# josef-w/Differentiable-iLQR

Hardware: AMD Instinct MI355X
Metric: iLQR iters/sec (whole node), batch=65536 cartpole T=25 at 1/2/4/8 MI355X (higher is better)
Workload: dtype f32; 1 GPU; cartpole n=5 m=1 T=25, unconstrained iLQR, 65536 problems per GPU, step = one whole-batch MPC solve of lqr_iter=10 from u=0; batch_per_gpu=65536, global_batch=65536, T=25, lqr_iter=10, parallelism=batch-sharded x1 (no collective)

## Files before the change

differentiable-ilqr_amd/csrc/dilqr_fused.h:

```cpp
#pragma once
#include "dilqr_common.h"
#include "dilqr_launch.h"

namespace dilqr {

constexpr int TRAJ_AOS = 0, TRAJ_REC = 1;

template <int TL, int n, int m>
DEV void ld_xu(float (&x)[n], float (&u)[m], const float* __restrict__ xp, const float* __restrict__ up, size_t t,
               int B, int b) {
  const size_t tb = t * B + b;
  if constexpr (TL == TRAJ_REC) {
    float r[n + m];
    ld(r, (xp + (size_t)b * (n + m)) + t * (size_t)B * (n + m));
#pragma unroll
    for (int i = 0; i < n; ++i) x[i] = r[i];
#pragma unroll
    for (int a = 0; a < m; ++a) u[a] = r[n + a];
  } else {
    ld(x, xp + tb * n);
    ld(u, up + tb * m);
  }
}

template <int TL, int n, int m>
DEV void st_xu(float* __restrict__ xp, float* __restrict__ up, const float (&x)[n], const float (&u)[m], size_t t,
               int B, int b) {
  const size_t tb = t * B + b;
  if constexpr (TL == TRAJ_REC) {
    float r[n + m];
#pragma unroll
    for (int i = 0; i < n; ++i) r[i] = x[i];
#pragma unroll
    for (int a = 0; a < m; ++a) r[n + a] = u[a];
    st(xp + tb * (n + m), r);
  } else {
    st(xp + tb * n, x);
    st(up + tb * m, u);
  }
}

template <int d>
struct CostFull {
  static constexpr bool kDiag = false;
  static constexpr bool kSym = false;
  const float* __restrict__ C;
  const float* __restrict__ c;
  DEV void load(float (&Cr)[d][d], float (&cr)[d], size_t t, int B, int b) const {
    const size_t tb = t * B + b;
    ld2(Cr, C + tb * d * d); ld(cr, c + tb * d);
  }
};

template <int d>
constexpr int packed_cost_floats() { return d * (d + 1) / 2 + d; }
template <int d>
constexpr bool packed_diag_ok() { return (2 * d) % 4 == 0; }

constexpr unsigned char kCostSym = 1, kCostDiag = 2, kCostTinv = 4;

template <int d>
DEV void pack_cost(const float (&C)[d][d], const float (&c)[d], float (&buf)[packed_cost_floats<d>()], bool& sym,
                   bool& diag) {
  int k = 0;
#pragma unroll
  for (int i = 0; i < d; ++i) buf[k++] = C[i][i];
#pragma unroll
  for (int i = 0; i < d; ++i) buf[k++] = c[i];
  unsigned asym = 0u, offd = 0u;
#pragma unroll
  for (int i = 0; i < d; ++i)
#pragma unroll
    for (int j = i + 1; j < d; ++j) {
      asym |= __float_as_uint(C[i][j]) ^ __float_as_uint(C[j][i]);
      offd |= __float_as_uint(C[i][j]) | __float_as_uint(C[j][i]);
      buf[k++] = C[i][j];
    }
  sym &= asym == 0u;
  diag &= offd == 0u;
}

template <int K>
DEV bool same_bits(const float (&a)[K], const float (&b)[K]) {
  unsigned dif = 0u;
#pragma unroll
  for (int k = 0; k < K; ++k) dif |= __float_as_uint(a[k]) ^ __float_as_uint(b[k]);
  return dif == 0u;
}

template <int d, bool DIAG = false, bool TINV = false>
struct CostPacked {
  static constexpr bool kDiag = DIAG;
  static constexpr bool kSym = true;
  const float* __restrict__ P;
  int T;
  DEV void load(float (&Cr)[d][d], float (&cr)[d], size_t t_, int B, int b) const {
    constexpr int PK = packed_cost_floats<d>();
    const size_t t = TINV ? (size_t)(T - 1) : t_;
    if constexpr (DIAG) {
      static_assert(packed_diag_ok<d>(), "diagonal read needs whole float4 planes");
      constexpr int Q4 = SoaRec<PK>::Q4;
      const float4* q = reinterpret_cast<const float4*>(P);
      float buf[2 * d];
#pragma unroll
      for (int j = 0; j < 2 * d / 4; ++j) {
        float4 v = q[(t * Q4 + j) * B + b];
        buf[4 * j] = v.x; buf[4 * j + 1] = v.y; buf[4 * j + 2] = v.z; buf[4 * j + 3] = v.w;
      }
      const float z = 0.f;
#pragma unroll
      for (int i = 0; i < d; ++i) {
#pragma unroll
        for (int j = 0; j < d; ++j) Cr[i][j] = z;
        Cr[i][i] = buf[i];
        cr[i] = buf[d + i];
      }
    } else {
      float buf[PK];
      SoaRec<PK>::load(buf, P, T, t, B, b);
      int k = 2 * d;
#pragma unroll
      for (int i = 0; i < d; ++i) {
        Cr[i][i] = buf[i];
        cr[i] = buf[d + i];
      }
#pragma unroll
      for (int i = 0; i < d; ++i)
#pragma unroll
        for (int j = i + 1; j < d; ++j) { Cr[i][j] = buf[k]; Cr[j][i] = buf[k]; ++k; }
    }
  }
};

template <int d>
struct CostDiagConst {
  static constexpr bool kDiag = true;
  static constexpr bool kSym = true;
  float dg[d], cc[d];
  DEV void init(const float* __restrict__ P, int T, int B, int b) {
    float Cr[d][d], cr[d];
    CostPacked<d, true>{P, T}.load(Cr, cr, T - 1, B, b);
#pragma unroll
    for (int i = 0; i < d; ++i) { dg[i] = Cr[i][i]; cc[i] = cr[i]; }
  }
  template <int PK>
  DEV void set(const float (&pk)[PK]) {
#pragma unroll
    for (int i = 0; i < d; ++i) { dg[i] = pk[i]; cc[i] = pk[d + i]; }
  }
  DEV void load(float (&Cr)[d][d], float (&cr)[d], size_t, int, int) const {
    const float z = 0.f;
#pragma unroll
    for (int i = 0; i < d; ++i) {
#pragma unroll
      for (int j = 0; j < d; ++j) Cr[i][j] = z;
      Cr[i][i] = dg[i];
      cr[i] = cc[i];
    }
  }
};

template <class Model>
struct LaneCarry {
  static constexpr int n = Model::N, m = Model::M, d = n + m;
  float x0[n];
  CostDiagConst<d> cc;
  float u0[m], x1[n], u1[m];
  float xl[n], ul[m];
};

template <int m, int BM>
struct StepBounds {
  float lo[m], hi[m];
  DEV void load(const Bounds& bd, int t, int B, int b) {
    if constexpr (BM == DILQR_BOUNDS_TENSOR) {
      const size_t tb = (size_t)t * B + b;
      ld(lo, bd.lo_t + tb * m); ld(hi, bd.hi_t + tb * m);
    }
  }
  DEV float l(const Bounds& bd, int a) const {
    if constexpr (BM == DILQR_BOUNDS_TENSOR) return lo[a];
    else return bd.lo;
  }
  DEV float h(const Bounds& bd, int a) const {
    if constexpr (BM == DILQR_BOUNDS_TENSOR) return hi[a];
    else return bd.hi;
  }
};

template <int n, int m, int TL, int BM>
struct SweepIn {
  static constexpr int d = n + m;
  float C[d][d], c[d], x[n], u[m];
  StepBounds<m, BM> bnd;
  template <class CostT>
  DEV void load(const CostT& cs, const float* __restrict__ xp, const float* __restrict__ up, const Bounds& bd, int t,
                int B, int b) {
    cs.load(C, c, t, B, b); ld_xu<TL>(x, u, xp, up, t, B, b); bnd.load(bd, t, B, b);
  }
  template <class CostT>
  DEV void load_carried(const CostT& cs, const float (&xr)[n], const float (&ur)[m], const Bounds& bd, int t, int B,
                        int b) {
    cs.load(C, c, t, B, b); bnd.load(bd, t, B, b);
#pragma unroll
    for (int i = 0; i < n; ++i) x[i] = xr[i];
#pragma unroll
    for (int a = 0; a < m; ++a) u[a] = ur[a];
  }
};

struct GainRecs {
  float* p;
  int B, b;
};

template <int n, int m, int GREC, int TL, int BM>
struct FwdIn {
  static constexpr int d = n + m;
  float g[GREC], u[m], C[d][d], c[d], xnext[n], unext[m];
  StepBounds<m, BM> bnd;
  template <class CostT>
  DEV void load(const GainRecs& gr, const float* __restrict__ up, const CostT& cs,
                const float* __restrict__ xp, const Bounds& bd, int T, int t, int t1, int B, int b) {
    SoaRec<GREC>::load(g, gr.p, T, t, gr.B, gr.b); cs.load(C, c, t, B, b); bnd.load(bd, t, B, b);
    if constexpr (TL == TRAJ_REC) {
      ld_xu<TL>(xnext, unext, xp, up, t1, B, b);
    } else {
      ld(u, up + ((size_t)t * B + b) * m);
      ld(xnext, xp + ((size_t)t1 * B + b) * n);
    }
  }
  template <class CostT, class Carry>
  DEV void load_head(const GainRecs& gr, const CostT& cs, const Bounds& bd, const Carry& cy, int T, int B, int b) {
    SoaRec<GREC>::load(g, gr.p, T, 0, gr.B, gr.b); cs.load(C, c, 0, B, b); bnd.load(bd, 0, B, b);
#pragma unroll
    for (int i = 0; i < n; ++i) xnext[i] = cy.x1[i];
#pragma unroll
    for (int a = 0; a < m; ++a) { unext[a] = cy.u1[a]; u[a] = cy.u0[a]; }
  }
};

#ifndef DILQR_PF
#define DILQR_PF 2
#endif
constexpr int kPF = DILQR_PF;
#ifndef DILQR_PF_LS
#define DILQR_PF_LS 1
#endif
constexpr int kPFL = DILQR_PF_LS;
static_assert(kPFL == 1 || kPFL == 2, "the line search prefetches one or two steps ahead");

#ifndef DILQR_COPY_K
#define DILQR_COPY_K 5
#endif
constexpr int kCopyK = DILQR_COPY_K;

template <class Model, int BM, int TL, class CostT, bool PAIR = false, bool CARRY = false>
DEV int line_search(int T, int B, int b, const Model md, const float* __restrict__ x_init, const CostT& cs,
                    const float* __restrict__ x, const float* __restrict__ u, const Bounds& bd, float decay,
                    int max_ls, const GainRecs& ws, float* __restrict__ xa_out,
                    float* __restrict__ ua_out, float* __restrict__ xb_out, float* __restrict__ ub_out,
                    float* __restrict__ du_sq, float old_cost, float& cost_out, float& alpha_out,
                    bool b_in_gains = false, LaneCarry<Model>* cy = nullptr) {
  constexpr int n = Model::N, m = Model::M, d = n + m;
  constexpr int GREC = m * n + m;
  static_assert(!CARRY || TL == TRAJ_REC, "the carry hands over whole [x_t; u_t] records");
  f2 tl[d];
  static_assert(TL != TRAJ_REC || GREC == d, "B records in the gain slots need m = 1");
  if constexpr (PAIR) {
    max_ls = 2;
    b_in_gains = true;
  }
  float alpha = 1.f, cost = 0.f;
  int win = 0;
  for (int p = 0; p < max_ls; p += 2) {
    const bool twoB = p + 1 < max_ls;
    const float aA = alpha, aB = alpha * decay;
    const f2 al = {aA, aB};
    f2 xp[n], dp[n];
    {
      float x0[n];
      if constexpr (CARRY) {
#pragma unroll
        for (int i = 0; i < n; ++i) x0[i] = cy->x0[i];
      } else {
        ld(x0, x_init + (size_t)b * n);
      }
#pragma unroll
      for (int i = 0; i < n; ++i) { xp[i] = f2{x0[i], x0[i]}; dp[i] = f2{0.f, 0.f}; }
      if constexpr (TL == TRAJ_AOS) {
        st(xa_out + (size_t)b * n, x0);
        if (twoB) st(xb_out + (size_t)b * n, x0);
      }
    }
    f2 cp = {0.f, 0.f};
    auto cl = [T](int s) { return s < T ? s : T - 1; };
    FwdIn<n, m, GREC, TL, BM> cur, n1, n2;
    if constexpr (CARRY) {
      cur.load_head(ws, cs, bd, *cy, T, B, b);
    } else {
      cur.load(ws, u, cs, x, bd, T, 0, cl(1), B, b);
      if constexpr (TL == TRAJ_REC) {
        float x0r[n];
        ld_xu<TL>(x0r, cur.u, x, u, 0, B, b);
      }
    }
    if constexpr (kPFL >= 2) {
      if (T > 1) n1.load(ws, u, cs, x, bd, T, 1, cl(2), B, b);
    }
    auto step = [&](int t, auto last_c, auto& c, auto& nx) {
      constexpr bool LAST = decltype(last_c)::value;
      if constexpr (!LAST) {
        if constexpr (kPFL >= 2) {
          if (t + 2 < T) n2.load(ws, u, cs, x, bd, T, t + 2, cl(t + 3), B, b);
        } else {
          nx.load(ws, u, cs, x, bd, T, t + 1, cl(t + 2), B, b);
        }
      }
      f2 nu[m];
#pragma unroll
      for (int a = 0; a < m; ++a) {
        f2 sp = {0.f, 0.f};
#pragma unroll
        for (int j = 0; j < n; ++j) sp += c.g[a * n + j] * dp[j];
        nu[a] = (sp + c.u[a]) + al * c.g[m * n + a];
        if constexpr (BM != DILQR_BOUNDS_NONE) {
          const float lo = c.bnd.l(bd, a), hi = c.bnd.h(bd, a);
          nu[a] = f2{eclamp(nu[a].x, lo, hi), eclamp(nu[a].y, lo, hi)};
        }
      }
      {
        float ua[m], ub[m];
#pragma unroll
        for (int a = 0; a < m; ++a) { ua[a] = nu[a].x; ub[a] = nu[a].y; }
        if constexpr (TL == TRAJ_REC) {
          float xa[n], xb[n];
#pragma unroll
          for (int i = 0; i < n; ++i) { xa[i] = xp[i].x; xb[i] = xp[i].y; }
          st_xu<TL>(xa_out, nullptr, xa, ua, t, B, b);
          if (twoB) {
            if (b_in_gains) {
              float rb[d];
#pragma unroll
              for (int i = 0; i < n; ++i) rb[i] = xb[i];
#pragma unroll
              for (int a = 0; a < m; ++a) rb[n + a] = ub[a];
              SoaRec<d>::store(ws.p, rb, T, t, ws.B, ws.b);
            } else {
              st_xu<TL>(xb_out, nullptr, xb, ub, t, B, b);
            }
          }
        } else {
          st(ua_out + ((size_t)t * B + b) * m, ua);
          if (twoB) st(ub_out + ((size_t)t * B + b) * m, ub);
        }
      }
      if (p == 0) {
#pragma unroll
        for (int a = 0; a < m; ++a) {
          float e = c.u[a] - nu[a].x;
          du_sq[((size_t)t * m + a) * B + b] = e * e;
        }
      }
      f2 tau[d];
#pragma unroll
      for (int i = 0; i < n; ++i) tau[i] = xp[i];
#pragma unroll
      for (int a = 0; a < m; ++a) tau[n + a] = nu[a];
      cp += quad_cost<d, CostT::kDiag>(c.C, c.c, tau);
      if constexpr (CARRY && LAST) {
#pragma unroll
        for (int i = 0; i < d; ++i) tl[i] = tau[i];
      }
      if constexpr (!LAST) {
        f2 xnext[n];
        md.forward(xp, nu, xnext);
        float xa[n], xb[n];
#pragma unroll
        for (int i = 0; i < n; ++i) {
          dp[i] = xnext[i] - c.xnext[i];
          xp[i] = xnext[i];
          xa[i] = xnext[i].x;
          xb[i] = xnext[i].y;
        }
        if constexpr (TL == TRAJ_AOS) {
          st(xa_out + ((size_t)(t + 1) * B + b) * n, xa);
          if (twoB) st(xb_out + ((size_t)(t + 1) * B + b) * n, xb);
        }
      }
      if constexpr (!LAST) {
        if constexpr (TL == TRAJ_REC) {
#pragma unroll
          for (int a = 0; a < m; ++a) nx.u[a] = c.unext[a];
        }
      }
    };
    for (int t = 0; t < T - 1; ++t) {
      step(t, std::false_type{}, cur, n1);
      cur = n1;
      if constexpr (kPFL >= 2) n1 = n2;
#ifdef DILQR_STAMPS
      if (t == 0) DILQR_STAMP(9);
#endif
    }
    step(T - 1, std::true_type{}, cur, n1);
    DILQR_STAMP(10);
    const float cA = cp.x, cB = cp.y;
    if (!(cA > old_cost) || p == max_ls - 1) { cost = cA; alpha = aA; win = 0; break; }
    if (!(cB > old_cost) || p + 1 == max_ls - 1) { cost = cB; alpha = aB; win = 1; break; }
    alpha = aB * decay;
  }
  if constexpr (CARRY) {
#pragma unroll
    for (int i = 0; i < n; ++i) cy->xl[i] = win ? tl[i].y : tl[i].x;
#pragma unroll
    for (int a = 0; a < m; ++a) cy->ul[a] = win ? tl[n + a].y : tl[n + a].x;
  }
  if constexpr (TL == TRAJ_REC) {
    if (b_in_gains && win == 1) {
      auto copy_steps = [&](int t0, auto k_c) {
        constexpr int K = decltype(k_c)::value;
        float rb[K][d];
#pragma unroll
        for (int k = 0; k < K; ++k) SoaRec<d>::load(rb[k], ws.p, T, t0 + k, ws.B, ws.b);
#pragma unroll
        for (int k = 0; k < K; ++k) {
          float xt[n], ut[m];
#pragma unroll
          for (int i = 0; i < n; ++i) xt[i] = rb[k][i];
#pragma unroll
          for (int a = 0; a < m; ++a) ut[a] = rb[k][n + a];
          st_xu<TL>(xb_out, nullptr, xt, ut, t0 + k, B, b);
        }
      };
      int t = 0;
      for (; t + kCopyK <= T; t += kCopyK) copy_steps(t, std::integral_constant<int, kCopyK>{});
      for (; t < T; ++t) copy_steps(t, std::integral_constant<int, 1>{});
    }
  }
  DILQR_STAMP(11);
  cost_out = cost;
  alpha_out = alpha;
  return win;
}

template <class Model, int BM, int TL, bool ROLLOUT, class CostT, bool PREV = false, bool CARRY = false>
DEV int ilqr_problem(int T, int B, int b, const Model md, const float* __restrict__ x_init, const CostT& cs,
                     float* __restrict__ pack_out, unsigned char* __restrict__ sym_out, const float* __restrict__ x,
                     const float* __restrict__ u, const Bounds& bd, float decay, int max_ls,
                     const GainRecs& ws, float* __restrict__ xa_out, float* __restrict__ ua_out,
                     float* __restrict__ xb_out, float* __restrict__ ub_out, float* __restrict__ du_sq,
                     float& cost_out, float& alpha_out, bool b_in_gains = false,
                     float prev_cost = 0.f, unsigned* flags_out = nullptr, LaneCarry<Model>* cy = nullptr) {
  constexpr int n = Model::N, m = Model::M, d = n + m;
  constexpr int MODE = BM == DILQR_BOUNDS_NONE ? GAIN_UNC : GAIN_BOX;
  constexpr int GREC = m * n + m;
  constexpr int PK = packed_cost_floats<d>();
  float old_cost = 0.f;
  if constexpr (PREV) old_cost = prev_cost;
  bool sym = true, diag = true, tinv = true;
  bool symsofar = true;
  float pk_last[PK];
  {
    RiccatiState<n, m> rs;
    rs.init();
    float xn[n];
#pragma unroll
    for (int i = 0; i < n; ++i) xn[i] = 0.f;
    SweepIn<n, m, TL, BM> cur, n1, n2;
    if constexpr (CARRY) cur.load_carried(cs, cy->xl, cy->ul, bd, T - 1, B, b);
    else cur.load(cs, x, u, bd, T - 1, B, b);
    if constexpr (kPF >= 2) n1.load(cs, x, u, bd, T > 1 ? T - 2 : 0, B, b);
    const int t_head = T > 1 ? 1 : 0;
    using SI = SweepIn<n, m, TL, BM>;
    auto sweep_body = [&](int t, auto last_c, const SI& cur, float (&g)[GREC]) {
      constexpr bool LAST = decltype(last_c)::value;
      float tau[d], Ctau[d], cb[d];
#pragma unroll
      for (int i = 0; i < n; ++i) tau[i] = cur.x[i];
#pragma unroll
      for (int a = 0; a < m; ++a) tau[n + a] = cur.u[a];
      if (pack_out) {
        float buf[PK];
        pack_cost(cur.C, cur.c, buf, sym, diag);
        if constexpr (LAST) {
          SoaRec<PK>::store(pack_out, buf, T, t, B, b);
#pragma unroll
          for (int k = 0; k < PK; ++k) pk_last[k] = buf[k];
        } else {
          const bool same = same_bits(buf, pk_last);
          if (tinv && !same)
            for (int s = t + 1; s < T - 1; ++s) SoaRec<PK>::store(pack_out, pk_last, T, s, B, b);
          tinv &= same;
          if (!tinv) SoaRec<PK>::store(pack_out, buf, T, t, B, b);
        }
      }
      float obj = 0.f;
      if constexpr (PREV) c_tau<d, CostT::kDiag>(cur.C, tau, Ctau);
      else obj = quad_cost<d, CostT::kDiag>(cur.C, cur.c, tau, Ctau);
#pragma unroll
      for (int i = 0; i < d; ++i) cb[i] = Ctau[i] + cur.c[i];
      float Ft[n][d];
      if constexpr (!LAST) {
        if constexpr (ROLLOUT && Model::kJacFromNext) md.jacobian_next(cur.x, cur.u, xn, Ft);
        else md.jacobian(cur.x, cur.u, Ft);
      } else {
#pragma unroll
        for (int i = 0; i < n; ++i)
#pragma unroll
          for (int j = 0; j < d; ++j) Ft[i][j] = 0.f;
      }
      float zIt[m], lb[m], ub[m];
#pragma unroll
      for (int a = 0; a < m; ++a) {
        zIt[a] = 0.f; lb[a] = 0.f; ub[a] = 0.f;
        if constexpr (MODE == GAIN_BOX) {
          lb[a] = cur.bnd.l(bd, a) - cur.u[a];
          ub[a] = cur.bnd.h(bd, a) - cur.u[a];
        }
      }
      float Kt[m][n], kt[m];
      using FS = typename Model::FSparsity;
      if constexpr (CostT::kSym) {
        rs.template step<MODE, FS, CostT::kDiag, true>(cur.C, cb, Ft, zIt, lb, ub, Kt, kt);
      } else {
        symsofar &= bitwise_symmetric(cur.C);
        if (symsofar) rs.template step<MODE, FS, CostT::kDiag, true>(cur.C, cb, Ft, zIt, lb, ub, Kt, kt);
        else rs.template step<MODE, FS, CostT::kDiag, false>(cur.C, cb, Ft, zIt, lb, ub, Kt, kt);
      }
#pragma unroll
      for (int a = 0; a < m; ++a) {
#pragma unroll
        for (int j = 0; j < n; ++j) g[a * n + j] = Kt[a][j];
        g[m * n + a] = kt[a];
      }
      if constexpr (!PREV) old_cost += obj;
#pragma unroll
      for (int i = 0; i < n; ++i) xn[i] = cur.x[i];
      if constexpr (CARRY) {
        if (t == t_head) {
#pragma unroll
          for (int i = 0; i < n; ++i) cy->x1[i] = cur.x[i];
#pragma unroll
          for (int a = 0; a < m; ++a) cy->u1[a] = cur.u[a];
        }
#pragma unroll
        for (int a = 0; a < m; ++a) cy->u0[a] = cur.u[a];
      }
    };
    auto sweep_step = [&](int t, auto last_c) {
      if constexpr (kPF >= 2) n2.load(cs, x, u, bd, t > 1 ? t - 2 : 0, B, b);
      else n1.load(cs, x, u, bd, t > 0 ? t - 1 : 0, B, b);
      float g[GREC];
      sweep_body(t, last_c, cur, g);
      SoaRec<GREC>::store(ws.p, g, T, t, ws.B, ws.b);
      cur = n1;
      if constexpr (kPF >= 2) n1 = n2;
    };
    sweep_step(T - 1, std::true_type{});
    DILQR_STAMP(8);
#ifndef DILQR_SWEEP_UNROLL
#define DILQR_SWEEP_UNROLL 2
#endif
#pragma unroll DILQR_SWEEP_UNROLL
    for (int t = T - 2; t >= 0; --t) sweep_step(t, std::false_type{});
    if constexpr (CARRY) {
#pragma unroll
      for (int i = 0; i < n; ++i) cy->x0[i] = xn[i];
    }
    if (sym_out) {
      const unsigned char f = sym ? (unsigned char)(kCostSym | (diag && packed_diag_ok<d>() ? kCostDiag : 0) |
                                                    (tinv ? kCostTinv : 0))
                                  : 0;
      sym_out[b] = f;
      if (flags_out) *flags_out = f;
    }
  }
  DILQR_STAMP(2);
  if constexpr (!CostT::kDiag && packed_diag_ok<d>()) {
    if (pack_out && sym && diag && tinv) {
      CostDiagConst<d> cc;
      cc.set(pk_last);
      if (b_in_gains && max_ls == 2)
        return line_search<Model, BM, TL, CostDiagConst<d>, true, CARRY>(T, B, b, md, x_init, cc, x, u, bd, decay,
                                                                         max_ls, ws, xa_out, ua_out, xb_out, ub_out,
                                                                         du_sq, old_cost, cost_out, alpha_out,
                                                                         b_in_gains, cy);
      return line_search<Model, BM, TL, CostDiagConst<d>, false, CARRY>(T, B, b, md, x_init, cc, x, u, bd, decay,
                                                                        max_ls, ws, xa_out, ua_out, xb_out, ub_out,
                                                                        du_sq, old_cost, cost_out, alpha_out,
                                                                        b_in_gains, cy);
    }
  }
  if (b_in_gains && max_ls == 2)
    return line_search<Model, BM, TL, CostT, true, CARRY>(T, B, b, md, x_init, cs, x, u, bd, decay, max_ls, ws, xa_out,
                                                          ua_out, xb_out, ub_out, du_sq, old_cost, cost_out,
                                                          alpha_out, b_in_gains, cy);
  return line_search<Model, BM, TL, CostT, false, CARRY>(T, B, b, md, x_init, cs, x, u, bd, decay, max_ls, ws, xa_out,
                                                         ua_out, xb_out, ub_out, du_sq, old_cost, cost_out, alpha_out,
                                                         b_in_gains, cy);
}

template <class Model, int BM>
__global__ void __launch_bounds__(kBlock) k_ilqr_iterate(int T, int B, const float* __restrict__ theta,
                                                         const float* __restrict__ x_init, const float* __restrict__ C,
                                                         const float* __restrict__ c, const float* __restrict__ x,
                                                         const float* __restrict__ u, Bounds bd, float decay, int max_ls,
                                                         float* __restrict__ ws, float* __restrict__ x_out,
                                                         float* __restrict__ u_out, float* __restrict__ cost_out,
                                                         float* __restrict__ du_sq, float* __restrict__ alpha_out,
                                                         const dilqr_mpc_ctrl* __restrict__ ctrl) {
  if (ctrl && ctrl->stopped) return;
  int b = blockIdx.x * blockDim.x + threadIdx.x;
  if (b >= B) return;
  constexpr int n = Model::N, m = Model::M;
  constexpr int GREC = m * n + m;
  Model md; md.load(theta);
  float cost, alpha;
  float* xb = ws + (size_t)T * B * GREC;
  float* ub = xb + (size_t)T * B * n;
  const int win = ilqr_problem<Model, BM, TRAJ_AOS, false>(T, B, b, md, x_init, CostFull<n + m>{C, c}, nullptr, nullptr, x, u,
                                                   bd, decay,
                                            max_ls, GainRecs{ws, B, b},
                                            x_out, u_out, xb, ub, du_sq, cost, alpha);
  if (win) {
    for (int t = 0; t < T; ++t) {
      const size_t tb = (size_t)t * B + b;
      float xt[n], ut[m];
      ld(xt, xb + tb * n); ld(ut, ub + tb * m);
      st(x_out + tb * n, xt); st(u_out + tb * m, ut);
    }
  }
  cost_out[b] = cost;
  alpha_out[b] = alpha;
}

using MpcState = dilqr_mpc_state;
constexpr int kSlots = 4;

DEV bool mpc_decide(const MpcState& S, int B, int k, int G, float eps, int not_improved_lim);

DEV void free_slots(int cur, int best, int& sa, int& sb) {
  sa = -1;
  sb = -1;
#pragma unroll
  for (int s = 0; s < kSlots; ++s) {
    const bool fr = s != cur && s != best;
    sb = (fr && sa >= 0 && sb < 0) ? s : sb;
    sa = (fr && sa < 0) ? s : sa;
  }
}

struct LaneIter {
  float cost, alpha;
  int slot;
};

template <class Model, int BM, bool LG, bool FIRST, bool PREV = true, int GS = kBlock, bool CARRY = false,
          bool ONLY_DC = false>
DEV LaneIter mpc_iteration_lane(int T, int B, int b, const Model md, const float* __restrict__ x_init,
                                const float* __restrict__ C, const float* __restrict__ c, const Bounds& bd,
                                float decay, int max_ls, const MpcState& S, float* __restrict__ du_sq,
                                float* __restrict__ lds_gains, int cur, int best, unsigned pk, float prev_cost,
                                unsigned* flags_out = nullptr, LaneCarry<Model>* cy = nullptr) {
  constexpr int n = Model::N, m = Model::M;
  const size_t TBd = (size_t)T * B * (n + m);
  int sa, sb;
  free_slots(cur, best, sa, sb);
  const float* xcur = S.Xs + cur * TBd;
  float* xsa = S.Xs + sa * TBd;
  float* xsb = S.Xs + sb * TBd;
  float cost, alpha;
  int win;
  const GainRecs gr = LG ? GainRecs{lds_gains, GS, (int)threadIdx.x} : GainRecs{S.ws, B, b};
  const CostFull<n + m> full{C, c};
  const bool b_lds = LG && max_ls <= 2;
  if constexpr (FIRST) {
    win = ilqr_problem<Model, BM, TRAJ_REC, true>(T, B, b, md, x_init, full, S.Cpk, S.Cpk ? S.cost_sym : nullptr,
                                                  xcur, nullptr, bd, decay, max_ls, gr, xsa, nullptr, xsb, nullptr,
                                                  du_sq, cost, alpha, b_lds, 0.f, flags_out);
  } else {
    if (ONLY_DC || (pk & (kCostDiag | kCostTinv)) == (kCostDiag | kCostTinv)) {
      if constexpr (packed_diag_ok<n + m>()) {
        CostDiagConst<n + m> cc;
        if constexpr (CARRY) cc = cy->cc;
        else cc.init(S.Cpk, T, B, b);
        win = ilqr_problem<Model, BM, TRAJ_REC, true, CostDiagConst<n + m>, PREV, CARRY>(T, B, b, md, x_init, cc, nullptr, nullptr, xcur, nullptr, bd,
                                                      decay, max_ls, gr, xsa, nullptr, xsb, nullptr, du_sq, cost,
                                                      alpha, b_lds, prev_cost, nullptr, cy);
      } else {
        __builtin_unreachable();
      }
    } else if constexpr (ONLY_DC) {
      __builtin_unreachable();
    } else if (pk & kCostDiag) {
      if constexpr (packed_diag_ok<n + m>())
        win = ilqr_problem<Model, BM, TRAJ_REC, true, CostPacked<n + m, true>, PREV, CARRY>(T, B, b, md, x_init, CostPacked<n + m, true>{S.Cpk, T}, nullptr,
                                                      nullptr, xcur, nullptr, bd, decay, max_ls, gr, xsa, nullptr, xsb,
                                                      nullptr, du_sq, cost, alpha, b_lds, prev_cost, nullptr, cy);
      else
        __builtin_unreachable();
    } else if ((pk & (kCostSym | kCostTinv)) == (kCostSym | kCostTinv))
      win = ilqr_problem<Model, BM, TRAJ_REC, true, CostPacked<n + m, false, true>, PREV, CARRY>(T, B, b, md, x_init, CostPacked<n + m, false, true>{S.Cpk, T},
                                                    nullptr, nullptr, xcur, nullptr, bd, decay, max_ls, gr, xsa, nullptr,
                                                    xsb, nullptr, du_sq, cost, alpha, b_lds, prev_cost, nullptr, cy);
    else if (pk & kCostSym)
      win = ilqr_problem<Model, BM, TRAJ_REC, true, CostPacked<n + m>, PREV, CARRY>(T, B, b, md, x_init, CostPacked<n + m>{S.Cpk, T}, nullptr, nullptr,
                                                    xcur, nullptr, bd, decay, max_ls, gr, xsa, nullptr, xsb, nullptr,
                                                    du_sq, cost, alpha, b_lds, prev_cost, nullptr, cy);
    else
      win = ilqr_problem<Model, BM, TRAJ_REC, true, CostFull<n + m>, PREV, CARRY>(T, B, b, md, x_init, full, nullptr, nullptr, xcur, nullptr, bd,
                                                    decay, max_ls, gr, xsa, nullptr, xsb, nullptr, du_sq, cost,
                                                    alpha, b_lds, prev_cost, nullptr, cy);
  }
  return LaneIter{cost, alpha, win ? sb : sa};
}

DEV bool mpc_takes_best(bool first, float cost, float best_cost, float best_cost_eps) {
  return first || cost <= best_cost + best_cost_eps;
}

template <class Model, int BM, bool LG, bool FIRST>
__global__ void __launch_bounds__(kBlock) k_mpc_iterate(int T, int B, const float* __restrict__ theta,
                                                        const float* __restrict__ x_init, const float* __restrict__ C,
                                                        const float* __restrict__ c, Bounds bd, float decay, int max_ls,
                                                        int iteration, float best_cost_eps, float eps,
                                                        int not_improved_lim, int G, MpcState S) {
  constexpr bool first = FIRST;
  int b = blockIdx.x * blockDim.x + threadIdx.x;
  const int bl = b < B ? b : B - 1;
  const int cur = S.slot[bl], best = S.slot[B + bl];
  const unsigned char pk = (!FIRST && S.Cpk) ? S.cost_sym[bl] : 0;
  const float prev = FIRST ? 0.f : S.cost[bl];
  const float best_cost = FIRST ? 0.f : S.best_cost[bl];
  DILQR_STAMP(0);
  DILQR_STAMP(6);
  if (mpc_decide(S, B, iteration, G, eps, not_improved_lim)) return;
  if (b >= B) return;
  DILQR_STAMP(1);
  Model md; md.load(theta);
  extern __shared__ __attribute__((aligned(16))) float lds_gains[];
  const LaneIter r = mpc_iteration_lane<Model, BM, LG, FIRST>(T, B, b, md, x_init, C, c, bd, decay, max_ls, S,
                                                              S.du_sq, lds_gains, cur, best, pk, prev);
  DILQR_STAMP(3);
  S.cost[b] = r.cost;
  S.alpha[b] = r.alpha;
  const bool take = mpc_takes_best(first, r.cost, best_cost, best_cost_eps);
  if (take) {
    S.best_cost[b] = r.cost;
    S.slot[B + b] = (unsigned char)r.slot;
  }
  S.improved[b] = take ? (first ? 1 : 2) : 0;
  if (S.best_iter && take) S.best_iter[b] = iteration;
  S.slot[b] = (unsigned char)r.slot;
  DILQR_STAMP(4);
  DILQR_STAMP(7);
}

DEV int sync_gmax(int B) { return (B + 63) / 64; }

DEV bool mpc_decide(const MpcState& S, int B, int k, int G, float eps, int not_improved_lim) {
  if (k == 0) return false;
  if (G < 0) return false;
  const int gm = sync_gmax(B), par = (k - 1) & 1;
  const unsigned* pm = S.done_counter + 16 + (2 * par) * gm;
  const unsigned* pa = S.done_counter + 16 + (2 * par + 1) * gm;
  const int lane = threadIdx.x & 63;
  const dilqr_mpc_ctrl in = S.ctrl[(k - 1) & 1];
  unsigned mx = 0u;
  int any = 0;
  if ((gm & 3) == 0 && G <= 1024) {
    const uint4* pm4 = reinterpret_cast<const uint4*>(pm);
    const uint4* pa4 = reinterpret_cast<const uint4*>(pa);
    uint4 vm[4], va[4];
#pragma unroll
    for (int j = 0; j < 4; ++j) {
      const int i = lane + 64 * j;
      const bool ok = 4 * i < G;
      vm[j] = ok ? pm4[i] : make_uint4(0u, 0u, 0u, 0u);
      va[j] = ok ? pa4[i] : make_uint4(0u, 0u, 0u, 0u);
    }
#pragma unroll
    for (int j = 0; j < 4; ++j) {
      const int i0 = 4 * (lane + 64 * j);
      const unsigned e[4] = {vm[j].x, vm[j].y, vm[j].z, vm[j].w};
      const unsigned f[4] = {va[j].x, va[j].y, va[j].z, va[j].w};
#pragma unroll
      for (int q = 0; q < 4; ++q) {
        if (i0 + q < G) {
          mx = e[q] > mx ? e[q] : mx;
          any |= (int)f[q];
        }
      }
    }
  } else {
    for (int i = lane; i < G; i += 64) {
      unsigned v = pm[i];
      mx = v > mx ? v : mx;
      any |= (int)pa[i];
    }
  }
  dilqr_mpc_ctrl out = in;
  if (!in.stopped) {
    const bool all_below = __ballot(!(__uint_as_float(mx) < eps)) == 0ull;
    const bool any_imp = __ballot(any != 0) != 0ull;
    out.iter = in.iter + 1;
    out.n_not_improved = any_imp ? 0 : in.n_not_improved + 1;
    if (all_below || out.n_not_improved > not_improved_lim) out.stopped = 1;
    if (blockIdx.x == 0) {
#pragma unroll
      for (int off = 32; off > 0; off >>= 1) {
        unsigned o = __shfl_xor(mx, off, 64);
        mx = o > mx ? o : mx;
      }
      out.max_du_bits = mx;
    }
  }
  if (blockIdx.x == 0 && threadIdx.x == 0) S.ctrl[k & 1] = out;
  return out.stopped != 0;
}

template <class Model>
constexpr int slot_layout() { return Model::N + Model::M <= 8 ? TRAJ_REC : TRAJ_AOS; }
constexpr int slot_layout_nm(int n, int m) { return n + m <= 8 ? TRAJ_REC : TRAJ_AOS; }

#ifndef DILQR_BEGIN_PF
#define DILQR_BEGIN_PF 1
#endif
template <class Model, bool ANALYSE = false, bool CARRY = false>
DEV unsigned mpc_begin_lane(int T, int B, int b, const Model& md, const float* __restrict__ x_init,
                            const float* __restrict__ u_init, const MpcState& S,
                            const float* __restrict__ C = nullptr, const float* __restrict__ c = nullptr,
                            LaneCarry<Model>* cy = nullptr) {
  constexpr int n = Model::N, m = Model::M, d = n + m;
  constexpr int PK = packed_cost_floats<d>();
  S.slot[b] = 0; S.slot[B + b] = 0;
  constexpr int TL = slot_layout<Model>();
  const CostFull<d> full{C, c};
  constexpr int PFB = ANALYSE ? DILQR_BEGIN_PF : 1;
  float Cq[PFB][d][d], cq[PFB][d], uq[PFB][m];
  auto load_step = [&](int s, int t) {
    if (u_init) {
      ld(uq[s], u_init + ((size_t)t * B + b) * m);
    } else {
#pragma unroll
      for (int a = 0; a < m; ++a) uq[s][a] = 0.f;
    }
    if constexpr (ANALYSE) full.load(Cq[s], cq[s], t, B, b);
  };
#pragma unroll
  for (int s = 0; s < PFB; ++s) load_step(s, s < T ? s : T - 1);
  bool sym = true, diag = true, tinv = true;
  float pk_first[PK];
  float xt[n];
  ld(xt, x_init + (size_t)b * n);
  for (int t0 = 0; t0 < T; t0 += PFB) {
#pragma unroll
    for (int s = 0; s < PFB; ++s) {
      const int t = t0 + s;
      if (t >= T) break;
      float ut[m], xn[n];
      float Cc[d][d], cc[d];
#pragma unroll
      for (int a = 0; a < m; ++a) ut[a] = uq[s][a];
      if constexpr (ANALYSE) {
#pragma unroll
        for (int i = 0; i < d; ++i) {
          cc[i] = cq[s][i];
#pragma unroll
          for (int j = 0; j < d; ++j) Cc[i][j] = Cq[s][i][j];
        }
      }
      const int tp = t + PFB < T ? t + PFB : T - 1;
      load_step(s, tp);
      st_xu<TL>(S.Xs, S.Us, xt, ut, t, B, b);
      if constexpr (CARRY) {
#pragma unroll
        for (int a = 0; a < m; ++a) cy->ul[a] = ut[a];
      }
      if (t < T - 1) {
        md.forward(xt, ut, xn);
#pragma unroll
        for (int i = 0; i < n; ++i) xt[i] = xn[i];
      }
      if constexpr (ANALYSE) {
        float buf[PK];
        pack_cost(Cc, cc, buf, sym, diag);
        if (t == 0) {
#pragma unroll
          for (int k = 0; k < PK; ++k) pk_first[k] = buf[k];
        } else {
          const bool same = same_bits(buf, pk_first);
          if (tinv && !same)
            for (int s_ = 0; s_ < t; ++s_) SoaRec<PK>::store(S.Cpk, pk_first, T, s_, B, b);
          tinv &= same;
          if (!tinv) SoaRec<PK>::store(S.Cpk, buf, T, t, B, b);
        }
      }
    }
  }
  if constexpr (CARRY) {
#pragma unroll
    for (int i = 0; i < n; ++i) cy->xl[i] = xt[i];
    if constexpr (ANALYSE && packed_diag_ok<d>()) cy->cc.set(pk_first);
  }
  if constexpr (ANALYSE) {
    if (tinv) SoaRec<PK>::store(S.Cpk, pk_first, T, T - 1, B, b);
    const unsigned char f = sym ? (unsigned char)(kCostSym | (diag && packed_diag_ok<d>() ? kCostDiag : 0) |
                                                  (tinv ? kCostTinv : 0))
                                : 0;
    S.cost_sym[b] = f;
    return f;
  }
  return 0u;
}

constexpr int kDenseCount = 9;

DEV void mpc_reset_ctrl(const MpcState& S) {
  dilqr_mpc_ctrl z = {};
  S.ctrl[0] = z;
  S.ctrl[1] = z;
#pragma unroll
  for (int i = 0; i <= kDenseCount; ++i) S.done_counter[i] = 0u;
}

#ifndef DILQR_SOLVE_LPW
#define DILQR_SOLVE_LPW 64
#endif
#ifndef DILQR_SOLVE_OCC
#define DILQR_SOLVE_OCC 1
#endif
constexpr int kSolveLpw = DILQR_SOLVE_LPW;

template <class Model, int BM, bool LG>
__global__ void __launch_bounds__(kBlock, DILQR_SOLVE_OCC) k_mpc_solve_fixed(int T, int B, const float* __restrict__ theta,
                                                            const float* __restrict__ x_init,
                                                            const float* __restrict__ u_init,
                                                            const float* __restrict__ C, const float* __restrict__ c,
                                                            Bounds bd, float decay, int max_ls, int iters,
                                                            float best_cost_eps, MpcState S) {
  constexpr int m = Model::M;
  const int b = blockIdx.x * kSolveLpw + threadIdx.x;
  DILQR_STAMP(0);
  DILQR_STAMP(6);
  if (b == 0) mpc_reset_ctrl(S);
  if (b >= B || (int)threadIdx.x >= kSolveLpw) return;
  Model md; md.load(theta);
  extern __shared__ __attribute__((aligned(16))) float lds_gains[];
  LaneCarry<Model> cy;
  const unsigned pk = S.Cpk ? mpc_begin_lane<Model, true, true>(T, B, b, md, x_init, u_init, S, C, c, &cy)
                            : mpc_begin_lane<Model, false, true>(T, B, b, md, x_init, u_init, S, nullptr, nullptr, &cy);
  DILQR_STAMP(1);
  LaneIter r{0.f, 0.f, 0};
  int cur = 0, best = 0, best_iter = 0;
  float best_cost = 0.f;
  bool take = true;
  const size_t plane = (size_t)T * m * B;
  auto iterate = [&](auto only_dc) {
    constexpr bool DC = decltype(only_dc)::value;
    r = mpc_iteration_lane<Model, BM, LG, false, false, kSolveLpw, true, DC>(T, B, b, md, x_init, C, c, bd, decay,
                                                                             max_ls, S, S.du_sq, lds_gains, 0, 0, pk,
                                                                             0.f, nullptr, &cy);
    cur = best = r.slot;
    best_cost = r.cost;
    DILQR_STAMP(3);
    for (int it = 1; it < iters; ++it) {
      if (it == iters - 1) DILQR_STAMP(4);
      r = mpc_iteration_lane<Model, BM, LG, false, true, kSolveLpw, true, DC>(T, B, b, md, x_init, C, c, bd, decay,
                                                                              max_ls, S, S.du_sq + it * plane,
                                                                              lds_gains, cur, best, pk, r.cost,
                                                                              nullptr, &cy);
      take = mpc_takes_best(false, r.cost, best_cost, best_cost_eps);
      if (take) { best_cost = r.cost; best = r.slot; best_iter = it; }
      cur = r.slot;
    }
  };
  bool wave_dc = false;
  if constexpr (packed_diag_ok<Model::N + m>())
    wave_dc = __ballot((pk & (kCostDiag | kCostTinv)) != (kCostDiag | kCostTinv)) == 0ull;
  if (wave_dc) iterate(std::true_type{});
  else iterate(std::false_type{});
  S.cost[b] = r.cost;
  S.alpha[b] = r.alpha;
  S.best_cost[b] = best_cost;
  S.slot[b] = (unsigned char)cur;
  S.slot[B + b] = (unsigned char)best;
  S.improved[b] = take ? (iters == 1 ? 1 : 2) : 0;
  S.best_iter[b] = best_iter;
  DILQR_STAMP(5);
  DILQR_STAMP(7);
}

constexpr int kSmallMax = 256;

template <class Model, int BM, bool LG>
__global__ void __launch_bounds__(kSmallMax) k_mpc_solve_small(int T, int B, const float* __restrict__ theta,
                                                               const float* __restrict__ x_init,
                                                               const float* __restrict__ u_init,
                                                               const float* __restrict__ C,
                                                               const float* __restrict__ c, Bounds bd, float decay,
                                                               int max_ls, int iters, float best_cost_eps, float eps,
                                                               int not_improved_lim, MpcState S) {
  constexpr int m = Model::M;
  __shared__ unsigned red_max[kSmallMax / 64];
  __shared__ int red_any[kSmallMax / 64];
  extern __shared__ __attribute__((aligned(16))) float lds_gains[];
  const int b = threadIdx.x;
  const bool act = b < B;
  const int nw = (int)(blockDim.x + 63) / 64, w = b >> 6;
  const int TM = T * m;
  Model md; md.load(theta);
  unsigned pk = 0u;
  LaneIter r{0.f, 0.f, 0};
  int cur = 0, best = 0, imp = 0;
  float best_cost = 0.f;
  if (act) {
    pk = S.Cpk ? mpc_begin_lane<Model, true>(T, B, b, md, x_init, u_init, S, C, c)
               : mpc_begin_lane<Model>(T, B, b, md, x_init, u_init, S);
    r = mpc_iteration_lane<Model, BM, LG, false, false, 64>(T, B, b, md, x_init, C, c, bd, decay, max_ls, S,
                                                            S.du_sq, lds_gains, 0, 0, pk, 0.f);
    cur = best = r.slot;
    best_cost = r.cost;
    imp = 1;
  }
  int done = 0, n_not_improved = 0, stopped = 0;
  unsigned mx_all = 0u, mx_prev = 0u;
  for (;;) {
    ++done;
    __syncthreads();
    unsigned mx = 0u;
    int any = 0;
    if (act) {
      float s2 = 0.f;
      const float* p = S.du_sq + (size_t)b * TM;
      for (int i = 0; i < TM; ++i) s2 += p[i];
      const float fdn = sqrtf(s2);
      S.full_du_norm[b] = fdn;
      if (imp) S.best_du[b] = fdn;
      mx = __float_as_uint(fdn);
      any = imp == 2;
    }
#pragma unroll
    for (int off = 32; off > 0; off >>= 1) {
      const unsigned o = __shfl_xor(mx, off, 64);
      mx = o > mx ? o : mx;
      any |= __shfl_xor(any, off, 64);
    }
    if ((b & 63) == 0) { red_max[w] = mx; red_any[w] = any; }
    __syncthreads();
    mx = 0u;
    any = 0;
    for (int i = 0; i < nw; ++i) { mx = red_max[i] > mx ? red_max[i] : mx; any |= red_any[i]; }
    mx_prev = mx_all;
    mx_all = mx;
    if (done == iters) break;
    n_not_improved = any ? 0 : n_not_improved + 1;
    if (__uint_as_float(mx) < eps || n_not_improved > not_improved_lim) {
      stopped = 1;
      break;
    }
    if (act) {
      r = mpc_iteration_lane<Model, BM, LG, false, true, 64>(T, B, b, md, x_init, C, c, bd, decay, max_ls, S,
                                                             S.du_sq, lds_gains, cur, best, pk, r.cost);
      const bool take = mpc_takes_best(false, r.cost, best_cost, best_cost_eps);
      if (take) { best_cost = r.cost; best = r.slot; }
      imp = take ? 2 : 0;
      cur = r.slot;
    }
  }
  if (act) {
    S.cost[b] = r.cost;
    S.alpha[b] = r.alpha;
    S.best_cost[b] = best_cost;
    S.slot[b] = (unsigned char)cur;
    S.slot[B + b] = (unsigned char)best;
    S.improved[b] = imp;
  }
  if (b == 0) {
    dilqr_mpc_ctrl o = {};
    o.iter = stopped ? done : done - 1;
    o.stopped = stopped;
    o.n_not_improved = n_not_improved;
    o.max_du_bits = stopped ? mx_all : mx_prev;
    S.ctrl[0] = o;
    S.ctrl[1] = o;
  }
}

inline bool lds_gains_fit(size_t lds, int B) {
  if (lds > 65536) return false;
  if (lds * 4 <= kLdsPerCU) return true;
  static int cus = [] {
    int dev = 0, n = 0;
    if (hipGetDevice(&dev) != hipSuccess ||
        hipDeviceGetAttribute(&n, hipDeviceAttributeMultiprocessorCount, dev) != hipSuccess)
      return 0;
    return n;
  }();
  return (size_t)grid_for(B) <= (size_t)cus * (kLdsPerCU / lds);
}
template <class MD>
int launch_mpc_step_tpp(const MpcStepArgs& a) {
#define LAUNCH_IT(BM_, LG_, FIRST_, LDS_)                                                                     \
  k_mpc_iterate<MD, BM_, LG_, FIRST_><<<grid_for(a.B), kBlock, LDS_, a.stream>>>(                            \
      a.T, a.B, a.theta, a.x_init, a.C, a.c, a.bd, a.decay, a.max_ls, a.iteration, a.best_cost_eps, a.eps, a.lim, \
      a.G, a.st)
#define LAUNCH_MPC(BM_)                                                                                      \
  do {                                                                                                       \
    const size_t lds = (size_t)a.T * kBlock * (MD::N * MD::M + MD::M) * sizeof(float);                      \
    const bool lg = lds_gains_fit(lds, a.B);                                                                 \
    if (a.iteration == 0 && lg) LAUNCH_IT(BM_, true, true, lds);                                             \
    else if (a.iteration == 0) LAUNCH_IT(BM_, false, true, 0);                                               \
    else if (lg) LAUNCH_IT(BM_, true, false, lds);                                                           \
    else LAUNCH_IT(BM_, false, false, 0);                                                                    \
  } while (0)
  if (a.bd.mode == DILQR_BOUNDS_TENSOR) LAUNCH_MPC(DILQR_BOUNDS_TENSOR);
  else if (a.bd.mode != DILQR_BOUNDS_NONE) LAUNCH_MPC(DILQR_BOUNDS_SCALAR);
  else LAUNCH_MPC(DILQR_BOUNDS_NONE);
#undef LAUNCH_MPC
#undef LAUNCH_IT
  return launched();
}

template <class MD>
int launch_mpc_solve_tpp(const MpcSolveArgs& a) {
#define LAUNCH_SOLVE(BM_)                                                                                    \
  do {                                                                                                       \
    const size_t lds = (size_t)a.T * kSolveLpw * (MD::N * MD::M + MD::M) * sizeof(float);                   \
    const int grid = (int)(((long long)a.B + kSolveLpw - 1) / kSolveLpw);                                   \
    if (lds_gains_fit(lds * kBlock / kSolveLpw, a.B))                                                       \
      k_mpc_solve_fixed<MD, BM_, true><<<grid, kBlock, lds, a.stream>>>(                                      \
          a.T, a.B, a.theta, a.x_init, a.u_init, a.C, a.c, a.bd, a.decay, a.max_ls, a.iters, a.best_cost_eps, a.st); \
    else                                                                                                     \
      k_mpc_solve_fixed<MD, BM_, false><<<grid, kBlock, 0, a.stream>>>(                                       \
          a.T, a.B, a.theta, a.x_init, a.u_init, a.C, a.c, a.bd, a.decay, a.max_ls, a.iters, a.best_cost_eps, a.st); \
  } while (0)
  if (a.bd.mode == DILQR_BOUNDS_TENSOR) LAUNCH_SOLVE(DILQR_BOUNDS_TENSOR);
  else if (a.bd.mode != DILQR_BOUNDS_NONE) LAUNCH_SOLVE(DILQR_BOUNDS_SCALAR);
  else LAUNCH_SOLVE(DILQR_BOUNDS_NONE);
#undef LAUNCH_SOLVE
  return launched();
}

template <class MD>
int launch_mpc_solve_small_tpp(const MpcSolveArgs& a, float eps, int lim) {
  if (a.B > kSmallMax) return DILQR_E_SHAPE;
  const int threads = (a.B + 63) / 64 * 64;
  const size_t lds = (size_t)a.T * 64 * (MD::N * MD::M + MD::M) * sizeof(float);
  const bool lg = threads == 64 && lds <= 65536;
#define LAUNCH_SMALL(BM_)                                                                                    \
  do {                                                                                                       \
    if (lg)                                                                                                  \
      k_mpc_solve_small<MD, BM_, true><<<1, threads, lds, a.stream>>>(                                        \
          a.T, a.B, a.theta, a.x_init, a.u_init, a.C, a.c, a.bd, a.decay, a.max_ls, a.iters, a.best_cost_eps, eps, \
          lim, a.st);                                                                                        \
    else                                                                                                     \
      k_mpc_solve_small<MD, BM_, false><<<1, threads, 0, a.stream>>>(                                         \
          a.T, a.B, a.theta, a.x_init, a.u_init, a.C, a.c, a.bd, a.decay, a.max_ls, a.iters, a.best_cost_eps, eps, \
          lim, a.st);                                                                                        \
  } while (0)
  if (a.bd.mode == DILQR_BOUNDS_TENSOR) LAUNCH_SMALL(DILQR_BOUNDS_TENSOR);
  else if (a.bd.mode != DILQR_BOUNDS_NONE) LAUNCH_SMALL(DILQR_BOUNDS_SCALAR);
  else LAUNCH_SMALL(DILQR_BOUNDS_NONE);
#undef LAUNCH_SMALL
  return launched();
}

template <class MD>
int launch_ilqr_iterate_tpp(const IlqrIterArgs& a) {
#define LAUNCH_IT(BM_)                                                                                        \
  k_ilqr_iterate<MD, BM_><<<grid_for(a.B), kBlock, 0, a.stream>>>(a.T, a.B, a.theta, a.x_init, a.C, a.c, a.x, a.u, \
                                                                   a.bd, a.decay, a.max_ls, a.ws, a.x_out,     \
                                                                   a.u_out, a.cost, a.du_sq, a.alpha, a.ctrl)
  if (a.bd.mode == DILQR_BOUNDS_TENSOR) LAUNCH_IT(DILQR_BOUNDS_TENSOR);
  else if (a.bd.mode != DILQR_BOUNDS_NONE) LAUNCH_IT(DILQR_BOUNDS_SCALAR);
  else LAUNCH_IT(DILQR_BOUNDS_NONE);
#undef LAUNCH_IT
  return launched();
}

}
```

Measured before the change: 2.009 billion problem-iters/s.

## Speculate diagonal time-invariant cost and verify lazily during backward sweeps

For the cartpole, unconstrained, LDS-gains path, the kernel now checks only the first and last cost records. If every lane in the wave has a diagonal, time-invariant cost, it skips the full cost-packing pass and runs the diagonal-constant iteration straight away. The remaining per-step cost records are loaded and compared a few at a time inside the sweep steps to hide the check's latency, and the packed cost is committed only if the whole wave passes. If verification fails, the whole solve is redone on the original path, which doubles the work for inputs that violate the assumption.

```diff
diff --git a/differentiable-ilqr_amd/csrc/dilqr_cost_check.h b/differentiable-ilqr_amd/csrc/dilqr_cost_check.h
--- /dev/null
+++ b/differentiable-ilqr_amd/csrc/dilqr_cost_check.h
@@ -0,0 +1,68 @@
+#pragma once
+#ifdef __HIPCC__
+#include "dilqr_device.h"
+#define DILQR_HD __host__ __device__ __forceinline__
+#else
+#define DILQR_HD inline
+#endif
+
+namespace dilqr {
+
+DILQR_HD unsigned f32_bits(float x) { return __builtin_bit_cast(unsigned, x); }
+
+template <int d>
+DILQR_HD unsigned cost_record_diff(const float (&C)[d][d], const float (&c)[d], const float (&dg)[d],
+                                   const float (&cc)[d]) {
+  unsigned x = 0u;
+#pragma unroll
+  for (int i = 0; i < d; ++i) {
+#pragma unroll
+    for (int j = 0; j < d; ++j) x |= i == j ? f32_bits(C[i][i]) ^ f32_bits(dg[i]) : f32_bits(C[i][j]);
+    x |= f32_bits(c[i]) ^ f32_bits(cc[i]);
+  }
+  return x;
+}
+
+struct SpecSchedule {
+  int last;
+  int loaded;
+  int folded;
+  int events;
+  int fired;
+  int ticks;
+  int acc;
+  static DILQR_HD int stagger(unsigned wave, int gap) {
+    return (int)(((wave * 2654435761u) >> 16) % (unsigned)gap);
+  }
+  DILQR_HD void init(int T, int iters, int spread, int ticks_per_iteration, unsigned wave) {
+    last = T - 2;
+    loaded = 0;
+    folded = 0;
+    const int its = spread < iters ? spread : iters;
+    ticks = its > 0 ? its * ticks_per_iteration : 0;
+    events = (T > 2 && ticks >= T - 1) ? T - 1 : 0;
+    fired = 0;
+    acc = ticks - events;
+    if (events > 0) acc -= stagger(wave, ticks / events) * events;
+  }
+  DILQR_HD bool tick() {
+    if (fired == events) return false;
+    acc += events;
+    if (acc < ticks) return false;
+    acc -= ticks;
+    ++fired;
+    return true;
+  }
+  DILQR_HD bool take_fold() {
+    if (folded == loaded) return false;
+    ++folded;
+    return true;
+  }
+  DILQR_HD int take_load() {
+    if (loaded >= last) return 0;
+    return ++loaded;
+  }
+  DILQR_HD bool done() const { return folded >= last; }
+};
+
+}
diff --git a/differentiable-ilqr_amd/csrc/dilqr_fused.h b/differentiable-ilqr_amd/csrc/dilqr_fused.h
--- a/differentiable-ilqr_amd/csrc/dilqr_fused.h
+++ b/differentiable-ilqr_amd/csrc/dilqr_fused.h
@@ -1,5 +1,6 @@
 #pragma once
 #include "dilqr_common.h"
+#include "dilqr_cost_check.h"
 #include "dilqr_launch.h"
 
 namespace dilqr {
@@ -160,6 +161,41 @@
   }
 };
 
+#ifndef DILQR_SPEC_SPREAD
+#define DILQR_SPEC_SPREAD (1 << 20)
+#endif
+constexpr int kSpecSpread = DILQR_SPEC_SPREAD;
+template <class Model>
+struct SpecCostRoute : std::false_type {};
+template <>
+struct SpecCostRoute<Cartpole> : std::true_type {};
+
+template <int d>
+struct CostCheck {
+  SpecSchedule sch;
+  const float* __restrict__ C;
+  const float* __restrict__ c;
+  unsigned bad;
+  float Cb[d][d], cb[d];
+  DEV void init(const float* __restrict__ C_, const float* __restrict__ c_, int T, int iters) {
+    C = C_; c = c_; bad = 0u;
+    sch.init(T, iters, kSpecSpread, T, blockIdx.x);
+  }
+  DEV void event(const CostDiagConst<d>& guess, int B, int b) {
+    if (sch.take_fold()) bad |= cost_record_diff(Cb, cb, guess.dg, guess.cc);
+    const int t = sch.take_load();
+    if (t) CostFull<d>{C, c}.load(Cb, cb, t, B, b);
+  }
+  DEV void drain(const CostDiagConst<d>& guess, int B, int b) {
+    if (sch.take_fold()) bad |= cost_record_diff(Cb, cb, guess.dg, guess.cc);
+    for (int t = sch.take_load(); t; t = sch.take_load()) {
+      CostFull<d>{C, c}.load(Cb, cb, t, B, b);
+      sch.take_fold();
+      bad |= cost_record_diff(Cb, cb, guess.dg, guess.cc);
+    }
+  }
+};
+
 template <class Model>
 struct LaneCarry {
   static constexpr int n = Model::N, m = Model::M, d = n + m;
@@ -167,6 +203,10 @@
   CostDiagConst<d> cc;
   float u0[m], x1[n], u1[m];
   float xl[n], ul[m];
+  CostCheck<d> chk;
+  DEV void spec_step(int B, int b) {
+    if (chk.sch.tick()) chk.event(cc, B, b);
+  }
 };
 
 template <int m, int BM>
@@ -444,7 +484,8 @@
   return win;
 }
 
-template <class Model, int BM, int TL, bool ROLLOUT, class CostT, bool PREV = false, bool CARRY = false>
+template <class Model, int BM, int TL, bool ROLLOUT, class CostT, bool PREV = false, bool CARRY = false,
+          bool SPEC = false>
 DEV int ilqr_problem(int T, int B, int b, const Model md, const float* __restrict__ x_init, const CostT& cs,
                      float* __restrict__ pack_out, unsigned char* __restrict__ sym_out, const float* __restrict__ x,
                      const float* __restrict__ u, const Bounds& bd, float decay, int max_ls,
@@ -549,6 +590,7 @@
       }
     };
     auto sweep_step = [&](int t, auto last_c) {
+      if constexpr (SPEC) cy->spec_step(B, b);
       if constexpr (kPF >= 2) n2.load(cs, x, u, bd, t > 1 ? t - 2 : 0, B, b);
       else n1.load(cs, x, u, bd, t > 0 ? t - 1 : 0, B, b);
       float g[GREC];
@@ -657,7 +699,7 @@
 };
 
 template <class Model, int BM, bool LG, bool FIRST, bool PREV = true, int GS = kBlock, bool CARRY = false,
-          bool ONLY_DC = false>
+          int ONLY_DC = 0>
 DEV LaneIter mpc_iteration_lane(int T, int B, int b, const Model md, const float* __restrict__ x_init,
                                 const float* __restrict__ C, const float* __restrict__ c, const Bounds& bd,
                                 float decay, int max_ls, const MpcState& S, float* __restrict__ du_sq,
@@ -680,18 +722,18 @@
                                                   xcur, nullptr, bd, decay, max_ls, gr, xsa, nullptr, xsb, nullptr,
                                                   du_sq, cost, alpha, b_lds, 0.f, flags_out);
   } else {
-    if (ONLY_DC || (pk & (kCostDiag | kCostTinv)) == (kCostDiag | kCostTinv)) {
+    if (ONLY_DC != 0 || (pk & (kCostDiag | kCostTinv)) == (kCostDiag | kCostTinv)) {
       if constexpr (packed_diag_ok<n + m>()) {
         CostDiagConst<n + m> cc;
         if constexpr (CARRY) cc = cy->cc;
         else cc.init(S.Cpk, T, B, b);
-        win = ilqr_problem<Model, BM, TRAJ_REC, true, CostDiagConst<n + m>, PREV, CARRY>(T, B, b, md, x_init, cc, nullptr, nullptr, xcur, nullptr, bd,
+        win = ilqr_problem<Model, BM, TRAJ_REC, true, CostDiagConst<n + m>, PREV, CARRY, ONLY_DC == 2>(T, B, b, md, x_init, cc, nullptr, nullptr, xcur, nullptr, bd,
                                                       decay, max_ls, gr, xsa, nullptr, xsb, nullptr, du_sq, cost,
                                                       alpha, b_lds, prev_cost, nullptr, cy);
       } else {
         __builtin_unreachable();
       }
-    } else if constexpr (ONLY_DC) {
+    } else if constexpr (ONLY_DC != 0) {
       __builtin_unreachable();
     } else if (pk & kCostDiag) {
       if constexpr (packed_diag_ok<n + m>())
@@ -949,16 +991,17 @@
   Model md; md.load(theta);
   extern __shared__ __attribute__((aligned(16))) float lds_gains[];
   LaneCarry<Model> cy;
-  const unsigned pk = S.Cpk ? mpc_begin_lane<Model, true, true>(T, B, b, md, x_init, u_init, S, C, c, &cy)
-                            : mpc_begin_lane<Model, false, true>(T, B, b, md, x_init, u_init, S, nullptr, nullptr, &cy);
-  DILQR_STAMP(1);
+  unsigned pk = 0u;
   LaneIter r{0.f, 0.f, 0};
   int cur = 0, best = 0, best_iter = 0;
   float best_cost = 0.f;
   bool take = true;
   const size_t plane = (size_t)T * m * B;
   auto iterate = [&](auto only_dc) {
-    constexpr bool DC = decltype(only_dc)::value;
+    constexpr int DC = decltype(only_dc)::value;
+    r = LaneIter{0.f, 0.f, 0};
+    best_iter = 0;
+    take = true;
     r = mpc_iteration_lane<Model, BM, LG, false, false, kSolveLpw, true, DC>(T, B, b, md, x_init, C, c, bd, decay,
                                                                              max_ls, S, S.du_sq, lds_gains, 0, 0, pk,
                                                                              0.f, nullptr, &cy);
@@ -976,11 +1019,50 @@
       cur = r.slot;
     }
   };
-  bool wave_dc = false;
-  if constexpr (packed_diag_ok<Model::N + m>())
-    wave_dc = __ballot((pk & (kCostDiag | kCostTinv)) != (kCostDiag | kCostTinv)) == 0ull;
-  if (wave_dc) iterate(std::true_type{});
-  else iterate(std::false_type{});
+  constexpr int d = Model::N + m;
+  bool committed = false;
+  if constexpr (BM == DILQR_BOUNDS_NONE && LG && SpecCostRoute<Model>::value && packed_diag_ok<d>()) {
+    bool spec = false;
+    if (S.Cpk) {
+      float C0[d][d], c0[d], Cl[d][d], cl[d];
+      const CostFull<d> full{C, c};
+      full.load(C0, c0, 0, B, b);
+      full.load(Cl, cl, T - 1, B, b);
+#pragma unroll
+      for (int i = 0; i < d; ++i) { cy.cc.dg[i] = C0[i][i]; cy.cc.cc[i] = c0[i]; }
+      const unsigned miss = cost_record_diff(C0, c0, cy.cc.dg, cy.cc.cc) | cost_record_diff(Cl, cl, cy.cc.dg, cy.cc.cc);
+      spec = __ballot(miss != 0u) == 0ull;
+    }
+    if (spec) {
+      mpc_begin_lane<Model, false, true>(T, B, b, md, x_init, u_init, S, nullptr, nullptr, &cy);
+      DILQR_STAMP(1);
+      cy.chk.init(C, c, T, iters);
+      pk = kCostSym | kCostDiag | kCostTinv;
+      iterate(std::integral_constant<int, 2>{});
+      cy.chk.drain(cy.cc, B, b);
+      if (__ballot(cy.chk.bad != 0u) == 0ull) {
+        constexpr int PK = packed_cost_floats<d>();
+        float rec[PK];
+#pragma unroll
+        for (int k = 0; k < PK; ++k) rec[k] = 0.f;
+#pragma unroll
+        for (int i = 0; i < d; ++i) { rec[i] = cy.cc.dg[i]; rec[d + i] = cy.cc.cc[i]; }
+        SoaRec<PK>::store(S.Cpk, rec, T, T - 1, B, b);
+        S.cost_sym[b] = (unsigned char)pk;
+        committed = true;
+      }
+    }
+  }
+  if (!committed) {
+    pk = S.Cpk ? mpc_begin_lane<Model, true, true>(T, B, b, md, x_init, u_init, S, C, c, &cy)
+               : mpc_begin_lane<Model, false, true>(T, B, b, md, x_init, u_init, S, nullptr, nullptr, &cy);
+    DILQR_STAMP(1);
+    bool wave_dc = false;
+    if constexpr (packed_diag_ok<d>())
+      wave_dc = __ballot((pk & (kCostDiag | kCostTinv)) != (kCostDiag | kCostTinv)) == 0ull;
+    if (wave_dc) iterate(std::integral_constant<int, 1>{});
+    else iterate(std::integral_constant<int, 0>{});
+  }
   S.cost[b] = r.cost;
   S.alpha[b] = r.alpha;
   S.best_cost[b] = best_cost;
```

New measurement: 2.047 billion problem-iters/s, median of 6. +1.9%, better.
